# Agent-Field/agentfield

Measured on AMD Instinct MI355X. Metric: reasoner_calls_per_sec, higher is better.
Workload: dtype bf16; 1 GPU; model=llama-3-8b, global_batch=128, seq_len=576, prompt_len=512, gen_len=64, parallelism=dp1, cp_workers=4, spec_steps=0, engine_proc=False

## Files before the change

agentfield_amd/csrc/attn_decode.hip:

```cpp
#include "common.h"

#define AD_D 128
#define AD_MAXG 8

template <int G, bool WIDE>
__global__ void __launch_bounds__(256) attn_decode_kernel(
    u16* __restrict__ out, float* __restrict__ po, float* __restrict__ pml,
    const u16* __restrict__ q, const u16* __restrict__ kc, const u16* __restrict__ vc,
    const i32* __restrict__ bt, const i32* __restrict__ len,
    float scale, int Hk, int page_size, int max_pages, int nsplit, i64 qs,
    int win) {
  const int b = blockIdx.x, kvh = blockIdx.y, split = blockIdx.z;
  const int wid = threadIdx.x >> 6, lane = threadIdx.x & 63;
  const int tg = lane >> 4, dl = lane & 15;
  const int Hq = Hk * G;

  const int L = len[b];
  const int s0 = (win > 0 && L > win) ? L - win : 0;
  const int chunk = (L - s0 + nsplit - 1) / nsplit;
  const int t0 = s0 + split * chunk;
  const int t1 = min(L, t0 + chunk);

  float qr[G][8];
#pragma unroll
  for (int g = 0; g < G; ++g) {
    const u16* qp = q + (size_t)b * qs + (kvh * G + g) * AD_D + dl * 8;
    s16x8 qv = *reinterpret_cast<const s16x8*>(qp);
#pragma unroll
    for (int j = 0; j < 8; ++j) qr[g][j] = bf2f((u16)qv[j]) * scale;
  }

  float m[G], l[G], acc[G][8];
#pragma unroll
  for (int g = 0; g < G; ++g) {
    m[g] = AF_NEG_INF;
    l[g] = 0.f;
#pragma unroll
    for (int j = 0; j < 8; ++j) acc[g][j] = 0.f;
  }

  const i32* btrow = bt + (size_t)b * max_pages;
  if (!WIDE) {
    for (int tb = t0 + wid * 4; tb < t1; tb += 16) {
      const int t = tb + tg;
      const bool valid = t < t1;
      const int tc = valid ? t : (t1 - 1);
      const i64 page = btrow[tc / page_size];
      const size_t base = (((size_t)page * Hk + kvh) * page_size +
                           (tc % page_size)) * AD_D + dl * 8;
      const s16x8 kv8 = *reinterpret_cast<const s16x8*>(kc + base);
      const s16x8 vv8 = *reinterpret_cast<const s16x8*>(vc + base);
      float kf[8], vf[8];
#pragma unroll
      for (int j = 0; j < 8; ++j) {
        kf[j] = bf2f((u16)kv8[j]);
        vf[j] = bf2f((u16)vv8[j]);
      }
#pragma unroll
      for (int g = 0; g < G; ++g) {
        float d = 0.f;
#pragma unroll
        for (int j = 0; j < 8; ++j) d += qr[g][j] * kf[j];
        float s = group16_sum_f32(d);
        if (!valid) s = AF_NEG_INF;
        float tm = fmaxf(s, __shfl_xor(s, 16, 64));
        tm = fmaxf(tm, __shfl_xor(tm, 32, 64));
        const float mn = fmaxf(m[g], tm);
        const float corr = (m[g] <= AF_NEG_INF) ? 0.f : __expf(m[g] - mn);
        const float p = (s <= AF_NEG_INF) ? 0.f : __expf(s - mn);
        float psum = p + __shfl_xor(p, 16, 64);
        psum += __shfl_xor(psum, 32, 64);
        l[g] = l[g] * corr + psum;
        m[g] = mn;
#pragma unroll
        for (int j = 0; j < 8; ++j)
          acc[g][j] = acc[g][j] * corr + p * vf[j];
      }
    }
  } else {
  auto tile_base = [&](int t) {
    const i64 page = btrow[t / page_size];
    return (((size_t)page * Hk + kvh) * page_size + (t % page_size)) * AD_D +
           dl * 8;
  };
  for (int tb = t0 + wid * 4; tb < t1; tb += 32) {
    const int ta = tb + tg, tb2 = tb + 16 + tg;
    const bool va = ta < t1, vb = tb2 < t1;
    const size_t base_a = tile_base(va ? ta : (t1 - 1));
    const size_t base_b = tile_base(vb ? tb2 : (t1 - 1));
    const s16x8 ka8 = *reinterpret_cast<const s16x8*>(kc + base_a);
    const s16x8 va8 = *reinterpret_cast<const s16x8*>(vc + base_a);
    const s16x8 kb8 = *reinterpret_cast<const s16x8*>(kc + base_b);
    const s16x8 vb8 = *reinterpret_cast<const s16x8*>(vc + base_b);
    float kfa[8], vfa[8], kfb[8], vfb[8];
#pragma unroll
    for (int j = 0; j < 8; ++j) {
      kfa[j] = bf2f((u16)ka8[j]);
      vfa[j] = bf2f((u16)va8[j]);
      kfb[j] = bf2f((u16)kb8[j]);
      vfb[j] = bf2f((u16)vb8[j]);
    }
#pragma unroll
    for (int half = 0; half < 2; ++half) {
      const bool valid = half ? vb : va;
      const float* kf = half ? kfb : kfa;
      const float* vf = half ? vfb : vfa;
#pragma unroll
      for (int g = 0; g < G; ++g) {
        float d = 0.f;
#pragma unroll
        for (int j = 0; j < 8; ++j) d += qr[g][j] * kf[j];
        float s = group16_sum_f32(d);
        if (!valid) s = AF_NEG_INF;
        float tm = fmaxf(s, __shfl_xor(s, 16, 64));
        tm = fmaxf(tm, __shfl_xor(tm, 32, 64));
        if (tm <= AF_NEG_INF) continue;
        const float mn = fmaxf(m[g], tm);
        const float corr = (m[g] <= AF_NEG_INF) ? 0.f : __expf(m[g] - mn);
        const float p = (s <= AF_NEG_INF) ? 0.f : __expf(s - mn);
        float psum = p + __shfl_xor(p, 16, 64);
        psum += __shfl_xor(psum, 32, 64);
        l[g] = l[g] * corr + psum;
        m[g] = mn;
#pragma unroll
        for (int j = 0; j < 8; ++j) acc[g][j] = acc[g][j] * corr + p * vf[j];
      }
    }
  }
  }
#pragma unroll
  for (int g = 0; g < G; ++g)
#pragma unroll
    for (int j = 0; j < 8; ++j) {
      acc[g][j] += __shfl_xor(acc[g][j], 16, 64);
      acc[g][j] += __shfl_xor(acc[g][j], 32, 64);
    }

  __shared__ float s_ml[4][G][2];
  __shared__ float s_o[4][G][AD_D];
  if (lane == 0) {
#pragma unroll
    for (int g = 0; g < G; ++g) { s_ml[wid][g][0] = m[g]; s_ml[wid][g][1] = l[g]; }
  }
  if (tg == 0) {
#pragma unroll
    for (int g = 0; g < G; ++g)
#pragma unroll
      for (int j = 0; j < 8; ++j) s_o[wid][g][dl * 8 + j] = acc[g][j];
  }
  __syncthreads();
  if (wid != 0) return;

#pragma unroll
  for (int g = 0; g < G; ++g) {
    float M = AF_NEG_INF;
#pragma unroll
    for (int w = 0; w < 4; ++w) M = fmaxf(M, s_ml[w][g][0]);
    float L2 = 0.f, o8[8];
#pragma unroll
    for (int j = 0; j < 8; ++j) o8[j] = 0.f;
#pragma unroll
    for (int w = 0; w < 4; ++w) {
      const float c = (s_ml[w][g][0] <= AF_NEG_INF) ? 0.f : __expf(s_ml[w][g][0] - M);
      L2 += s_ml[w][g][1] * c;
#pragma unroll
      for (int j = 0; j < 8; ++j) o8[j] += s_o[w][g][dl * 8 + j] * c;
    }
    if (tg != 0) continue;
    if (nsplit == 1) {
      const float inv = (L2 > 0.f) ? 1.f / L2 : 0.f;
      u16* op = out + (size_t)b * (Hq * AD_D) + (kvh * G + g) * AD_D + dl * 8;
      s16x8 ov;
#pragma unroll
      for (int j = 0; j < 8; ++j) ov[j] = (short)f2bf(o8[j] * inv);
      *reinterpret_cast<s16x8*>(op) = ov;
    } else {
      const size_t pbase = ((((size_t)b * Hk + kvh) * nsplit + split) * G + g);
      float* od = po + pbase * AD_D + dl * 8;
#pragma unroll
      for (int j = 0; j < 8; ++j) od[j] = o8[j];
      if (lane == 0) { pml[pbase * 2] = M; pml[pbase * 2 + 1] = L2; }
    }
  }
}

__global__ void __launch_bounds__(64) attn_decode_combine_kernel(
    u16* __restrict__ out, const float* __restrict__ po, const float* __restrict__ pml,
    int Hq, int G, int nsplit) {
  const int b = blockIdx.x, h = blockIdx.y;
  const int kvh = h / G, g = h % G;
  const int Hk = Hq / G;
  const int d0 = threadIdx.x * 2;

  float M = AF_NEG_INF;
  for (int s = 0; s < nsplit; ++s) {
    const size_t pbase = ((((size_t)b * Hk + kvh) * nsplit + s) * G + g);
    M = fmaxf(M, pml[pbase * 2]);
  }
  float L2 = 0.f, o0 = 0.f, o1 = 0.f;
  for (int s = 0; s < nsplit; ++s) {
    const size_t pbase = ((((size_t)b * Hk + kvh) * nsplit + s) * G + g);
    const float pm = pml[pbase * 2];
    const float c = (pm <= AF_NEG_INF) ? 0.f : __expf(pm - M);
    L2 += pml[pbase * 2 + 1] * c;
    o0 += po[pbase * AD_D + d0] * c;
    o1 += po[pbase * AD_D + d0 + 1] * c;
  }
  const float inv = (L2 > 0.f) ? 1.f / L2 : 0.f;
  u16* op = out + (size_t)b * (Hq * AD_D) + h * AD_D + d0;
  op[0] = f2bf(o0 * inv);
  op[1] = f2bf(o1 * inv);
}

AF_EXPORT int af_attn_decode(void* out, void* po, void* pml, const void* q,
                             const void* kc, const void* vc, const void* bt,
                             const void* len, float scale, int B, int Hq, int Hk,
                             int D, int page_size, int max_pages, int nsplit,
                             i64 qs, int win, void* stream) {
  if (D != AD_D) return 9002;
  const int G = Hq / Hk;
  if (G < 1 || G > AD_MAXG || G * Hk != Hq) return 9003;
  if (B == 0) return 0;
  dim3 grid(B, Hk, nsplit), blk(256);
  hipStream_t st = (hipStream_t)stream;
  const bool wide = (size_t)B * Hk * nsplit >= 1024;
#define AF_LAUNCH(GG)                                                            \
  do {                                                                           \
    if (wide)                                                                    \
      attn_decode_kernel<GG, true><<<grid, blk, 0, st>>>(                        \
          (u16*)out, (float*)po, (float*)pml, (const u16*)q, (const u16*)kc,     \
          (const u16*)vc, (const i32*)bt, (const i32*)len, scale, Hk,            \
          page_size, max_pages, nsplit, qs, win);                                \
    else                                                                         \
      attn_decode_kernel<GG, false><<<grid, blk, 0, st>>>(                       \
          (u16*)out, (float*)po, (float*)pml, (const u16*)q, (const u16*)kc,     \
          (const u16*)vc, (const i32*)bt, (const i32*)len, scale, Hk,            \
          page_size, max_pages, nsplit, qs, win);                                \
  } while (0)
  switch (G) {
    case 1: AF_LAUNCH(1); break;
    case 2: AF_LAUNCH(2); break;
    case 4: AF_LAUNCH(4); break;
    case 8: AF_LAUNCH(8); break;
    default: return 9003;
  }
#undef AF_LAUNCH
  if (nsplit > 1) {
    dim3 g2(B, Hq), b2(64);
    attn_decode_combine_kernel<<<g2, b2, 0, st>>>(
        (u16*)out, (const float*)po, (const float*)pml, Hq, G, nsplit);
  }
  return af_last_err();
}
```

Before: 81.28 calls/s.

## Software-pipeline paged decode attention with shared block table and DPP reductions

Restructures the decode attention kernel into a double-buffered loop that issues the next tile's K/V loads before computing the current tile. Block-table entries are staged in shared memory, with power-of-two page indexing replacing division. Q is staged in LDS instead of registers, row reductions use DPP, and occupancy hints are set per group size. The WIDE/narrow split is replaced by a FAST path chosen on page size and table capacity. This adds an extra __syncthreads and LDS use, and turns off FP contraction, which may change rounding.

```diff
diff --git a/agentfield_amd/csrc/attn_decode.hip b/agentfield_amd/csrc/attn_decode.hip
--- a/agentfield_amd/csrc/attn_decode.hip
+++ b/agentfield_amd/csrc/attn_decode.hip
@@ -2,16 +2,52 @@
 
 #define AD_D 128
 #define AD_MAXG 8
-
-template <int G, bool WIDE>
-__global__ void __launch_bounds__(256) attn_decode_kernel(
+#define AD_BT_CAP 2048
+
+template <int CTRL>
+__device__ __forceinline__ float ad_dpp_add(float v) {
+  const int o = __builtin_amdgcn_update_dpp(0, __float_as_int(v), CTRL, 0xf,
+                                            0xf, true);
+  return v + __int_as_float(o);
+}
+
+__device__ __forceinline__ float ad_row16_sum(float v) {
+  v = ad_dpp_add<0x128>(v);
+  v = ad_dpp_add<0x124>(v);
+  v = ad_dpp_add<0x4E>(v);
+  v = ad_dpp_add<0xB1>(v);
+  return v;
+}
+
+typedef __attribute__((ext_vector_type(4))) uint32_t ad_u32x4;
+
+__device__ __forceinline__ void ad_cvt8(const s16x8& r, float* f) {
+  const ad_u32x4 w = __builtin_bit_cast(ad_u32x4, r);
+#pragma unroll
+  for (int j = 0; j < 4; ++j) {
+    f[2 * j] = __uint_as_float(w[j] << 16);
+    f[2 * j + 1] = __uint_as_float(w[j] & 0xffff0000u);
+  }
+}
+
+template <int G, bool FAST>
+__global__ void __launch_bounds__(256)
+__attribute__((amdgpu_waves_per_eu(G <= 4 ? 4 : 2, G <= 4 ? 4 : 2)))
+attn_decode_kernel(
     u16* __restrict__ out, float* __restrict__ po, float* __restrict__ pml,
     const u16* __restrict__ q, const u16* __restrict__ kc, const u16* __restrict__ vc,
     const i32* __restrict__ bt, const i32* __restrict__ len,
     float scale, int Hk, int page_size, int max_pages, int nsplit, i64 qs,
     int win) {
+#pragma clang fp contract(off)
+  __shared__ float s_ml[4][G][2];
+  __shared__ float s_o[4][G][AD_D];
+  __shared__ __attribute__((aligned(16))) float s_q[G * AD_D];
+  __shared__ i32 s_bt[FAST ? AD_BT_CAP : 1];
+
   const int b = blockIdx.x, kvh = blockIdx.y, split = blockIdx.z;
-  const int wid = threadIdx.x >> 6, lane = threadIdx.x & 63;
+  const int wid = __builtin_amdgcn_readfirstlane(threadIdx.x >> 6);
+  const int lane = threadIdx.x & 63;
   const int tg = lane >> 4, dl = lane & 15;
   const int Hq = Hk * G;
 
@@ -21,13 +57,12 @@
   const int t0 = s0 + split * chunk;
   const int t1 = min(L, t0 + chunk);
 
-  float qr[G][8];
-#pragma unroll
-  for (int g = 0; g < G; ++g) {
-    const u16* qp = q + (size_t)b * qs + (kvh * G + g) * AD_D + dl * 8;
-    s16x8 qv = *reinterpret_cast<const s16x8*>(qp);
-#pragma unroll
-    for (int j = 0; j < 8; ++j) qr[g][j] = bf2f((u16)qv[j]) * scale;
+  if (threadIdx.x < G * 16) {
+    const u16* qa = q + (size_t)b * qs + kvh * G * AD_D + threadIdx.x * 8;
+    const s16x8 qv = *reinterpret_cast<const s16x8*>(qa);
+#pragma unroll
+    for (int j = 0; j < 8; ++j)
+      s_q[threadIdx.x * 8 + j] = bf2f((u16)qv[j]) * scale;
   }
 
   float m[G], l[G], acc[G][8];
@@ -40,94 +75,106 @@
   }
 
   const i32* btrow = bt + (size_t)b * max_pages;
-  if (!WIDE) {
-    for (int tb = t0 + wid * 4; tb < t1; tb += 16) {
-      const int t = tb + tg;
-      const bool valid = t < t1;
-      const int tc = valid ? t : (t1 - 1);
-      const i64 page = btrow[tc / page_size];
-      const size_t base = (((size_t)page * Hk + kvh) * page_size +
-                           (tc % page_size)) * AD_D + dl * 8;
-      const s16x8 kv8 = *reinterpret_cast<const s16x8*>(kc + base);
-      const s16x8 vv8 = *reinterpret_cast<const s16x8*>(vc + base);
-      float kf[8], vf[8];
-#pragma unroll
-      for (int j = 0; j < 8; ++j) {
-        kf[j] = bf2f((u16)kv8[j]);
-        vf[j] = bf2f((u16)vv8[j]);
+  if (t0 < t1) {
+    const int sh = __builtin_ctz(page_size), pmask = page_size - 1;
+    const int p_lo = t0 >> sh;
+    if (FAST) {
+      const int p_n = ((t1 - 1) >> sh) - p_lo + 1;
+      for (int i = threadIdx.x; i < p_n; i += 256) s_bt[i] = btrow[p_lo + i];
+    }
+    __syncthreads();
+
+    int tb = t0 + wid * 4;
+    if (tb < t1) {
+      const int tl = t1 - 1;
+      int tn = tb + tg;
+      const uint32_t page_stride = (uint32_t)(Hk * page_size * AD_D);
+      const uint32_t lane_off = (uint32_t)(kvh * page_size * AD_D + dl * 8);
+
+      auto issue = [&](s16x8& k8, s16x8& v8) {
+        const int c = min(tn, tl);
+        uint32_t pg, o;
+        if (FAST) {
+          pg = s_bt[(c >> sh) - p_lo];
+          o = c & pmask;
+        } else {
+          const int i = c / page_size;
+          pg = btrow[i];
+          o = c - i * page_size;
+        }
+        const size_t e = (size_t)pg * page_stride + (o * AD_D + lane_off);
+        k8 = *reinterpret_cast<const s16x8*>(kc + e);
+        v8 = *reinterpret_cast<const s16x8*>(vc + e);
+        tn += 16;
+      };
+
+      auto tile = [&](int t, const s16x8& k8, const s16x8& v8) {
+        const bool valid = t < t1;
+        float kf[8], s[G];
+        ad_cvt8(k8, kf);
+        asm volatile("" ::: "memory");
+#pragma unroll
+        for (int g = 0; g < G; ++g) {
+          const f32x4 q0 = *reinterpret_cast<const f32x4*>(s_q + g * AD_D + dl * 8);
+          const f32x4 q1 = *reinterpret_cast<const f32x4*>(s_q + g * AD_D + dl * 8 + 4);
+          float d = __builtin_fmaf(q0[0], kf[0], 0.f);
+          d = __builtin_fmaf(q0[1], kf[1], d);
+          d = d + q0[2] * kf[2];
+          d = d + q0[3] * kf[3];
+          d = d + q1[0] * kf[4];
+          d = d + q1[1] * kf[5];
+          d = d + q1[2] * kf[6];
+          d = d + q1[3] * kf[7];
+          const float r = ad_row16_sum(d);
+          s[g] = valid ? r : AF_NEG_INF;
+        }
+        float p[G], corr[G];
+#pragma unroll
+        for (int g = 0; g < G; ++g) {
+          float tm = fmaxf(s[g], __shfl_xor(s[g], 16, 64));
+          tm = fmaxf(tm, __shfl_xor(tm, 32, 64));
+          const float mn = fmaxf(m[g], tm);
+          corr[g] = (m[g] <= AF_NEG_INF) ? 0.f : __expf(m[g] - mn);
+          p[g] = (s[g] <= AF_NEG_INF) ? 0.f : __expf(s[g] - mn);
+          float psum = p[g] + __shfl_xor(p[g], 16, 64);
+          psum = psum + __shfl_xor(psum, 32, 64);
+          l[g] = __builtin_fmaf(l[g], corr[g], psum);
+          m[g] = mn;
+        }
+        const ad_u32x4 wv = __builtin_bit_cast(ad_u32x4, v8);
+#pragma unroll
+        for (int jj = 0; jj < 4; ++jj) {
+            const f32x2 v2 = {__uint_as_float(wv[jj] << 16),
+                            __uint_as_float(wv[jj] & 0xffff0000u)};
+#pragma unroll
+          for (int g = 0; g < G; ++g) {
+            const f32x2 pv = f32x2{p[g], p[g]} * v2;
+            const f32x2 o = __builtin_elementwise_fma(
+                f32x2{acc[g][2 * jj], acc[g][2 * jj + 1]},
+                f32x2{corr[g], corr[g]}, pv);
+            acc[g][2 * jj] = o[0];
+            acc[g][2 * jj + 1] = o[1];
+          }
+        }
+      };
+
+      s16x8 k0, v0, k1, v1;
+      issue(k0, v0);
+      while (tb + 16 < t1) {
+        issue(k1, v1);
+        __builtin_amdgcn_sched_barrier(0);
+        tile(tb + tg, k0, v0);
+        __builtin_amdgcn_sched_barrier(0);
+        issue(k0, v0);
+        __builtin_amdgcn_sched_barrier(0);
+        tile(tb + 16 + tg, k1, v1);
+        __builtin_amdgcn_sched_barrier(0);
+        tb += 32;
       }
-#pragma unroll
-      for (int g = 0; g < G; ++g) {
-        float d = 0.f;
-#pragma unroll
-        for (int j = 0; j < 8; ++j) d += qr[g][j] * kf[j];
-        float s = group16_sum_f32(d);
-        if (!valid) s = AF_NEG_INF;
-        float tm = fmaxf(s, __shfl_xor(s, 16, 64));
-        tm = fmaxf(tm, __shfl_xor(tm, 32, 64));
-        const float mn = fmaxf(m[g], tm);
-        const float corr = (m[g] <= AF_NEG_INF) ? 0.f : __expf(m[g] - mn);
-        const float p = (s <= AF_NEG_INF) ? 0.f : __expf(s - mn);
-        float psum = p + __shfl_xor(p, 16, 64);
-        psum += __shfl_xor(psum, 32, 64);
-        l[g] = l[g] * corr + psum;
-        m[g] = mn;
-#pragma unroll
-        for (int j = 0; j < 8; ++j)
-          acc[g][j] = acc[g][j] * corr + p * vf[j];
-      }
-    }
-  } else {
-  auto tile_base = [&](int t) {
-    const i64 page = btrow[t / page_size];
-    return (((size_t)page * Hk + kvh) * page_size + (t % page_size)) * AD_D +
-           dl * 8;
-  };
-  for (int tb = t0 + wid * 4; tb < t1; tb += 32) {
-    const int ta = tb + tg, tb2 = tb + 16 + tg;
-    const bool va = ta < t1, vb = tb2 < t1;
-    const size_t base_a = tile_base(va ? ta : (t1 - 1));
-    const size_t base_b = tile_base(vb ? tb2 : (t1 - 1));
-    const s16x8 ka8 = *reinterpret_cast<const s16x8*>(kc + base_a);
-    const s16x8 va8 = *reinterpret_cast<const s16x8*>(vc + base_a);
-    const s16x8 kb8 = *reinterpret_cast<const s16x8*>(kc + base_b);
-    const s16x8 vb8 = *reinterpret_cast<const s16x8*>(vc + base_b);
-    float kfa[8], vfa[8], kfb[8], vfb[8];
-#pragma unroll
-    for (int j = 0; j < 8; ++j) {
-      kfa[j] = bf2f((u16)ka8[j]);
-      vfa[j] = bf2f((u16)va8[j]);
-      kfb[j] = bf2f((u16)kb8[j]);
-      vfb[j] = bf2f((u16)vb8[j]);
-    }
-#pragma unroll
-    for (int half = 0; half < 2; ++half) {
-      const bool valid = half ? vb : va;
-      const float* kf = half ? kfb : kfa;
-      const float* vf = half ? vfb : vfa;
-#pragma unroll
-      for (int g = 0; g < G; ++g) {
-        float d = 0.f;
-#pragma unroll
-        for (int j = 0; j < 8; ++j) d += qr[g][j] * kf[j];
-        float s = group16_sum_f32(d);
-        if (!valid) s = AF_NEG_INF;
-        float tm = fmaxf(s, __shfl_xor(s, 16, 64));
-        tm = fmaxf(tm, __shfl_xor(tm, 32, 64));
-        if (tm <= AF_NEG_INF) continue;
-        const float mn = fmaxf(m[g], tm);
-        const float corr = (m[g] <= AF_NEG_INF) ? 0.f : __expf(m[g] - mn);
-        const float p = (s <= AF_NEG_INF) ? 0.f : __expf(s - mn);
-        float psum = p + __shfl_xor(p, 16, 64);
-        psum += __shfl_xor(psum, 32, 64);
-        l[g] = l[g] * corr + psum;
-        m[g] = mn;
-#pragma unroll
-        for (int j = 0; j < 8; ++j) acc[g][j] = acc[g][j] * corr + p * vf[j];
-      }
-    }
-  }
-  }
+      if (tb < t1) tile(tb + tg, k0, v0);
+    }
+  }
+
 #pragma unroll
   for (int g = 0; g < G; ++g)
 #pragma unroll
@@ -136,8 +183,6 @@
       acc[g][j] += __shfl_xor(acc[g][j], 32, 64);
     }
 
-  __shared__ float s_ml[4][G][2];
-  __shared__ float s_o[4][G][AD_D];
   if (lane == 0) {
 #pragma unroll
     for (int g = 0; g < G; ++g) { s_ml[wid][g][0] = m[g]; s_ml[wid][g][1] = l[g]; }
@@ -162,9 +207,10 @@
 #pragma unroll
     for (int w = 0; w < 4; ++w) {
       const float c = (s_ml[w][g][0] <= AF_NEG_INF) ? 0.f : __expf(s_ml[w][g][0] - M);
-      L2 += s_ml[w][g][1] * c;
-#pragma unroll
-      for (int j = 0; j < 8; ++j) o8[j] += s_o[w][g][dl * 8 + j] * c;
+      L2 = __builtin_fmaf(s_ml[w][g][1], c, L2);
+#pragma unroll
+      for (int j = 0; j < 8; ++j)
+        o8[j] = __builtin_fmaf(s_o[w][g][dl * 8 + j], c, o8[j]);
     }
     if (tg != 0) continue;
     if (nsplit == 1) {
@@ -223,10 +269,10 @@
   if (B == 0) return 0;
   dim3 grid(B, Hk, nsplit), blk(256);
   hipStream_t st = (hipStream_t)stream;
-  const bool wide = (size_t)B * Hk * nsplit >= 1024;
+  const bool fast = (page_size & (page_size - 1)) == 0 && max_pages <= AD_BT_CAP;
 #define AF_LAUNCH(GG)                                                            \
   do {                                                                           \
-    if (wide)                                                                    \
+    if (fast)                                                                    \
       attn_decode_kernel<GG, true><<<grid, blk, 0, st>>>(                        \
           (u16*)out, (float*)po, (float*)pml, (const u16*)q, (const u16*)kc,     \
           (const u16*)vc, (const i32*)bt, (const i32*)len, scale, Hk,            \
```

Result: faster. 85.26 calls/s, median of 6 (+4.9%).
